# zju3dv/Diffuman4D

Measured on NVIDIA H100. Metric: unet_window_denoise_steps_per_sec, higher is better.
Workload: dtype bf16

## Files before the change

diffuman4d_b200/csrc/common.cuh:

```cuda
#pragma once
#include <cuda.h>
#include <cuda_bf16.h>
#include <cuda_runtime.h>
#include <stdint.h>
#include <string>

namespace d4d {

typedef __nv_bfloat16 bf16;

void set_error(const std::string& msg);
#define D4D_CUDA_OK(expr)                                                                        \
  do {                                                                                           \
    cudaError_t _e = (expr);                                                                     \
    if (_e != cudaSuccess) {                                                                     \
      d4d::set_error(std::string(#expr) + " failed: " + cudaGetErrorString(_e) + " @" + __FILE__ + \
                     ":" + std::to_string(__LINE__));                                            \
      return 2;                                                                                  \
    }                                                                                            \
  } while (0)
#define D4D_REQUIRE(cond, msg)                                                                   \
  do {                                                                                           \
    if (!(cond)) {                                                                               \
      d4d::set_error(std::string("invalid argument: ") + msg + " (" #cond ") @" + __FILE__ + ":" + \
                     std::to_string(__LINE__));                                                  \
      return 1;                                                                                  \
    }                                                                                            \
  } while (0)

int make_tmap_2d(CUtensorMap* out, const void* base, uint64_t rows, uint64_t cols, uint64_t ld,
                 uint32_t box_cols, uint32_t box_rows, int swizzle_bytes);
int make_tmap_nhwc(CUtensorMap* out, const void* base, uint64_t n, uint64_t h, uint64_t w, uint64_t c,
                   uint32_t box_c, uint32_t box_w, uint32_t box_h, uint32_t box_n, int swizzle_bytes, int stride = 1);

#ifdef __CUDACC__
__device__ __forceinline__ uint32_t smem_u32(const void* p) {
  return static_cast<uint32_t>(__cvta_generic_to_shared(p));
}
__device__ __forceinline__ bool elect_one() {
  uint32_t pred = 0;
  asm volatile(
      "{\n\t.reg .b32 rx;\n\t.reg .pred px;\n\t"
      "elect.sync rx|px, 0xffffffff;\n\t"
      "selp.b32 %0, 1, 0, px;\n\t}\n"
      : "=r"(pred));
  return pred != 0;
}

__device__ __forceinline__ void mbar_init(uint64_t* bar, uint32_t count) {
  asm volatile("mbarrier.init.shared::cta.b64 [%0], %1;" ::"r"(smem_u32(bar)), "r"(count) : "memory");
}
__device__ __forceinline__ void fence_mbar_init() {
  asm volatile("fence.mbarrier_init.release.cluster;" ::: "memory");
}
__device__ __forceinline__ void mbar_expect_tx(uint64_t* bar, uint32_t bytes) {
  asm volatile("mbarrier.arrive.expect_tx.shared::cta.b64 _, [%0], %1;" ::"r"(smem_u32(bar)), "r"(bytes)
               : "memory");
}
__device__ __forceinline__ void mbar_arrive(uint64_t* bar) {
  asm volatile("mbarrier.arrive.shared::cta.b64 _, [%0];" ::"r"(smem_u32(bar)) : "memory");
}
__device__ __forceinline__ bool mbar_try_wait(uint64_t* bar, uint32_t parity) {
  uint32_t ok;
  asm volatile(
      "{\n\t.reg .pred p;\n\t"
      "mbarrier.try_wait.parity.shared::cta.b64 p, [%1], %2;\n\t"
      "selp.b32 %0, 1, 0, p;\n\t}\n"
      : "=r"(ok)
      : "r"(smem_u32(bar)), "r"(parity)
      : "memory");
  return ok != 0;
}
#ifndef D4D_SPIN_LIMIT
#define D4D_SPIN_LIMIT (1u << 26)
#endif
__device__ __forceinline__ void mbar_wait(uint64_t* bar, uint32_t parity) {
  uint32_t spins = 0;
  while (!mbar_try_wait(bar, parity)) {
    if (++spins > D4D_SPIN_LIMIT) {
      printf("d4d: mbarrier timeout block=(%d,%d) thread=%d bar=%u parity=%u\n", blockIdx.x, blockIdx.y,
             threadIdx.x, smem_u32(bar), parity);
      __trap();
    }
  }
}

__device__ __forceinline__ void fence_proxy_async_smem() {
  asm volatile("fence.proxy.async.shared::cta;" ::: "memory");
}
__device__ __forceinline__ void named_barrier_sync(int id, int threads) {
  asm volatile("bar.sync %0, %1;" ::"r"(id), "r"(threads) : "memory");
}
__device__ __forceinline__ void st_shared_u32(uint32_t addr, uint32_t v) {
  asm volatile("st.shared.b32 [%0], %1;" ::"r"(addr), "r"(v) : "memory");
}
__device__ __forceinline__ uint32_t ld_shared_u32(uint32_t addr) {
  uint32_t v;
  asm volatile("ld.shared.b32 %0, [%1];" : "=r"(v) : "r"(addr) : "memory");
  return v;
}
__device__ __forceinline__ void pdl_wait() { asm volatile("griddepcontrol.wait;" ::: "memory"); }
__device__ __forceinline__ void pdl_launch_dependents() { asm volatile("griddepcontrol.launch_dependents;" ::: "memory"); }
template <int R> __device__ __forceinline__ void setmaxnreg_dec() { asm volatile("setmaxnreg.dec.sync.aligned.u32 %0;" ::"n"(R)); }
template <int R> __device__ __forceinline__ void setmaxnreg_inc() { asm volatile("setmaxnreg.inc.sync.aligned.u32 %0;" ::"n"(R)); }

__device__ __forceinline__ void tma_prefetch_desc(const CUtensorMap* t) {
  asm volatile("prefetch.tensormap [%0];" ::"l"(reinterpret_cast<uint64_t>(t)) : "memory");
}
__device__ __forceinline__ void tma_load_2d(void* dst, const CUtensorMap* t, uint64_t* bar, int c0, int c1) {
  asm volatile(
      "cp.async.bulk.tensor.2d.shared::cluster.global.tile.mbarrier::complete_tx::bytes [%0], [%1, {%3, %4}], [%2];"
      ::"r"(smem_u32(dst)), "l"(reinterpret_cast<uint64_t>(t)), "r"(smem_u32(bar)), "r"(c0), "r"(c1)
      : "memory");
}
__device__ __forceinline__ void tma_load_4d(void* dst, const CUtensorMap* t, uint64_t* bar, int c0, int c1, int c2,
                                            int c3) {
  asm volatile(
      "cp.async.bulk.tensor.4d.shared::cluster.global.tile.mbarrier::complete_tx::bytes [%0], [%1, {%3, %4, %5, %6}], [%2];"
      ::"r"(smem_u32(dst)), "l"(reinterpret_cast<uint64_t>(t)), "r"(smem_u32(bar)), "r"(c0), "r"(c1), "r"(c2),
      "r"(c3)
      : "memory");
}

__device__ __forceinline__ void tma_store_2d(const CUtensorMap* t, const void* src, int c0, int c1) {
  asm volatile("cp.async.bulk.tensor.2d.global.shared::cta.bulk_group [%0, {%2, %3}], [%1];"
               ::"l"(reinterpret_cast<uint64_t>(t)), "r"(smem_u32(src)), "r"(c0), "r"(c1) : "memory");
}
__device__ __forceinline__ void bulk_commit_group() { asm volatile("cp.async.bulk.commit_group;" ::: "memory"); }
template <int N> __device__ __forceinline__ void bulk_wait_group_read() {
  asm volatile("cp.async.bulk.wait_group.read %0;" ::"n"(N) : "memory");
}
template <int N> __device__ __forceinline__ void bulk_wait_group() {
  asm volatile("cp.async.bulk.wait_group %0;" ::"n"(N) : "memory");
}

__device__ __forceinline__ uint32_t pack_bf16x2(float lo, float hi) {
  __nv_bfloat162 v = __floats2bfloat162_rn(lo, hi);
  return *reinterpret_cast<uint32_t*>(&v);
}
__device__ __forceinline__ float2 unpack_bf16x2(uint32_t u) {
  __nv_bfloat162 v = *reinterpret_cast<__nv_bfloat162*>(&u);
  return __bfloat1622float2(v);
}
__device__ __forceinline__ float silu_f(float x) { return __fdividef(x, 1.0f + __expf(-x)); }
__device__ __forceinline__ float gelu_erf_f(float g) {
  const float u = fabsf(g);
  float q = fmaf(-4.8811754095e-04f, u, 7.1988063864e-03f);
  q = fmaf(q, u, -5.2146803588e-02f);
  q = fmaf(q, u, -4.5959571004e-01f);
  q = fmaf(q, u, -1.1510006189e+00f);
  float e;
  asm("ex2.approx.ftz.f32 %0, %1;" : "=f"(e) : "f"(q * u));
  return fmaf(-0.5f * u, e, fmaxf(g, 0.f));
}
#endif

}
```

diffuman4d_b200/csrc/gemm_wgmma.cu:

```cuda
#include "kernels.h"
#include "wgmma.cuh"

namespace d4d {

namespace {

constexpr int BLOCK_M = 128;
constexpr int BLOCK_K = 64;
constexpr int A_BYTES = BLOCK_M * BLOCK_K * 2;
constexpr int BAR_BYTES = 1024;
constexpr int NUM_THREADS = 384;
constexpr int MAX_SMEM = 227 * 1024;

constexpr int SLAB_COLS = 32;
constexpr int SLAB_BYTES = 64 * SLAB_COLS * 2;

template <int BN, bool kStaged>
struct GemmCfg {
  static constexpr int STAGE_BYTES = A_BYTES + BN * BLOCK_K * 2;
  static constexpr int STAGING_BYTES = kStaged ? 2 * 64 * BN * 2 : 0;
  static constexpr int STAGES_FIT = (MAX_SMEM - 1024 - BAR_BYTES - STAGING_BYTES) / STAGE_BYTES;
  static constexpr int STAGES = STAGES_FIT > 8 ? 8 : STAGES_FIT;
  static constexpr int SMEM = 1024 + BAR_BYTES + STAGES * STAGE_BYTES + STAGING_BYTES;
};

struct TileCoord {
  int m0;
  int n_img0, y0, x0;
  int pa, pb;
};

template <bool kConv>
__device__ __forceinline__ void tile_coords(const GemmKernelArgs& a, int m_tile, TileCoord& t) {
  if (!kConv) {
    t.m0 = m_tile * BLOCK_M;
    t.n_img0 = t.y0 = t.x0 = 0;
    t.pa = t.pb = 0;
  } else {
    const int ph = a.n_phases > 1 ? m_tile / a.tiles_per_phase : 0;
    m_tile -= ph * a.tiles_per_phase;
    t.pa = ph >> 1;
    t.pb = ph & 1;
    int tx = m_tile % a.tiles_x;
    int r = m_tile / a.tiles_x;
    int ty = r % a.tiles_y;
    int tn = r / a.tiles_y;
    t.m0 = 0;
    t.x0 = tx * a.BW;
    t.y0 = ty * a.BH;
    t.n_img0 = tn * a.BN;
  }
}

template <bool kConv>
__device__ __forceinline__ void row_of(const GemmKernelArgs& a, const TileCoord& tc, int rr, long long& row, int& img,
                                       bool& valid) {
  if (!kConv) {
    row = static_cast<long long>(tc.m0) + rr;
    valid = row < a.M;
    img = a.rows_per_image > 0 ? static_cast<int>(row / a.rows_per_image) : 0;
  } else {
    const int bx = rr % a.BW;
    const int r2 = rr / a.BW;
    const int by = r2 % a.BH;
    const int bn = r2 / a.BH;
    const int x = tc.x0 + bx, y = tc.y0 + by, n = tc.n_img0 + bn;
    valid = (x < a.W) && (y < a.H) && (n < a.n_img);
    row = (static_cast<long long>(n) * a.out_H + (y * a.out_sy + a.out_oy + tc.pa)) * a.out_W + (x * a.out_sx + a.out_ox + tc.pb);
    img = n;
  }
}

enum : int { E_BIAS = 1, E_ROWVEC = 2, E_ACT = 4, E_RES = 8, E_STATS = 16, E_KV = 32, E_ALL = 63 };
__host__ __device__ constexpr bool gemm_staged(bool conv, int epi) { return !conv && !(epi & E_KV); }

template <int BN, bool kGeglu, bool kConv, int kEpi>
__global__ void __launch_bounds__(NUM_THREADS, 1)
gemm_wgmma_kernel(const __grid_constant__ CUtensorMap tmap_a, const __grid_constant__ CUtensorMap tmap_a2,
                  const __grid_constant__ CUtensorMap tmap_b, const __grid_constant__ CUtensorMap tmap_c,
                  const __grid_constant__ CUtensorMap tmap_r, const GemmKernelArgs a) {
  constexpr bool kStaged = gemm_staged(kConv, kEpi);
  using Cfg = GemmCfg<BN, kStaged>;
  constexpr int STAGES = Cfg::STAGES;
  extern __shared__ uint8_t smem_raw[];
  uint8_t* smem = reinterpret_cast<uint8_t*>((reinterpret_cast<uintptr_t>(smem_raw) + 1023) & ~uintptr_t(1023));
  uint64_t* full = reinterpret_cast<uint64_t*>(smem);
  uint64_t* empty = full + STAGES;
  uint64_t* res_full = empty + STAGES;
  uint8_t* ring = smem + BAR_BYTES;

  const int warp = __shfl_sync(0xffffffffu, threadIdx.x >> 5, 0);
  const int lane = threadIdx.x & 31;
  const int total_tiles = a.m_tiles * a.n_tiles;

  if (threadIdx.x == 0) {
    tma_prefetch_desc(&tmap_a);
    tma_prefetch_desc(&tmap_b);
    if (a.kb_split < a.k_blocks) tma_prefetch_desc(&tmap_a2);
    for (int i = 0; i < STAGES; ++i) {
      mbar_init(&full[i], 1);
      mbar_init(&empty[i], 2);
    }
    mbar_init(&res_full[0], 1);
    mbar_init(&res_full[1], 1);
    fence_mbar_init();
  }
  __syncthreads();
  pdl_wait();
  pdl_launch_dependents();

  if (warp < 4) {
    setmaxnreg_dec<40>();
    if (threadIdx.x == 0) {
      const uint32_t tx_bytes = A_BYTES + static_cast<uint32_t>(a.block_n) * BLOCK_K * 2;
      int stage = 0;
      uint32_t phase = 0;
      for (int tile = blockIdx.x; tile < total_tiles; tile += gridDim.x) {
        const int m_tile = tile / a.n_tiles;
        const int n_tile = tile % a.n_tiles;
        TileCoord tc;
        tile_coords<kConv>(a, m_tile, tc);
        const int n0 = n_tile * a.block_n;
        for (int kb = 0; kb < a.k_blocks; ++kb) {
          mbar_wait(&empty[stage], phase ^ 1);
          uint8_t* sa = ring + stage * Cfg::STAGE_BYTES;
          uint8_t* sb = sa + A_BYTES;
          mbar_expect_tx(&full[stage], tx_bytes);
          if (!kConv) {
            if (kb < a.kb_split) tma_load_2d(sa, &tmap_a, &full[stage], kb * BLOCK_K, tc.m0);
            else tma_load_2d(sa, &tmap_a2, &full[stage], (kb - a.kb_split) * BLOCK_K, tc.m0);
            tma_load_2d(sb, &tmap_b, &full[stage], kb * BLOCK_K, n0);
          } else {
            const int tap = kb / a.cin_blocks;
            const int cb = kb - tap * a.cin_blocks;
            tma_load_4d(sa, &tmap_a, &full[stage], cb * BLOCK_K, tc.x0 * a.in_stride + a.tap_dx[tap] + tc.pb,
                        tc.y0 * a.in_stride + a.tap_dy[tap] + tc.pa, tc.n_img0);
            tma_load_2d(sb, &tmap_b, &full[stage], tap * a.Cin + cb * BLOCK_K, n0 + (tc.pa * 2 + tc.pb) * a.N);
          }
          if (++stage == STAGES) { stage = 0; phase ^= 1; }
        }
      }
    }
    return;
  }

  setmaxnreg_inc<232>();
  const int wg = (warp >> 2) - 1;
  const int wq = warp & 3;
  const bool wg_leader = (threadIdx.x & 127) == 0;
  const int r_base = wg * 64 + wq * 16 + (lane >> 2);
  const int c_base = 2 * (lane & 3);
  const uint32_t ring_u32 = smem_u32(ring);
  const bool staged = kStaged && a.staged;
  uint8_t* stg = ring + STAGES * Cfg::STAGE_BYTES + wg * 64 * BN * 2;
  const uint32_t stg_u32 = smem_u32(stg) + (r_base - wg * 64) * 64 + c_base * 2;
  const int stg_xor = (lane >> 3) & 3;
  const bool has_res = (kEpi & E_RES) && !kGeglu && a.residual != nullptr;
  const int out_cols = kGeglu ? a.N / 2 : a.N;
  uint32_t res_phase = 0;

  int stage = 0;
  uint32_t phase = 0;
  float acc[BN / 2];
  for (int tile = blockIdx.x; tile < total_tiles; tile += gridDim.x) {
    const int m_tile = tile / a.n_tiles;
    const int n_tile = tile % a.n_tiles;
    TileCoord tc;
    tile_coords<kConv>(a, m_tile, tc);
    const int n0 = n_tile * a.block_n;
    const int ocol0 = kGeglu ? n0 / 2 : n0;
    const int ocols = min(kGeglu ? a.block_n / 2 : a.block_n, out_cols - ocol0);
    const int n_slabs = (ocols + SLAB_COLS - 1) / SLAB_COLS;
    const int orow0 = tc.m0 + wg * 64;
    const bool stg_live = staged && orow0 < a.M;

    int prev_stage = -1;
    for (int kb = 0; kb < a.k_blocks; ++kb) {
      mbar_wait(&full[stage], phase);
      const uint32_t sa = ring_u32 + stage * Cfg::STAGE_BYTES + wg * 64 * 128;
      const uint32_t sb = ring_u32 + stage * Cfg::STAGE_BYTES + A_BYTES;
      const uint64_t adesc = make_wgmma_desc(sa, 16, 1024);
      const uint64_t bdesc = make_wgmma_desc(sb, 16, 1024);
      wgmma_fence();
#pragma unroll
      for (int k = 0; k < BLOCK_K / 16; ++k) {
        const int scale_d = (kb | k) != 0 ? 1 : 0;
        if constexpr (BN == 64) wgmma_ss_n64(acc, adesc + 2 * k, bdesc + 2 * k, scale_d);
        else if constexpr (BN == 128) wgmma_ss_n128(acc, adesc + 2 * k, bdesc + 2 * k, scale_d);
        else if constexpr (BN == 160) wgmma_ss_n160(acc, adesc + 2 * k, bdesc + 2 * k, scale_d);
        else if constexpr (BN == 192) wgmma_ss_n192(acc, adesc + 2 * k, bdesc + 2 * k, scale_d);
        else wgmma_ss_n256(acc, adesc + 2 * k, bdesc + 2 * k, scale_d);
      }
      wgmma_commit();
      if (kb == 0 && staged && wg_leader) {
        bulk_wait_group_read<0>();
        if (has_res && stg_live) {
          mbar_expect_tx(&res_full[wg], n_slabs * SLAB_BYTES);
          for (int s = 0; s < n_slabs; ++s)
            tma_load_2d(stg + s * SLAB_BYTES, &tmap_r, &res_full[wg], ocol0 + s * SLAB_COLS, orow0);
        }
      }
      wgmma_wait<1>();
      if (prev_stage >= 0 && wg_leader) mbar_arrive(&empty[prev_stage]);
      prev_stage = stage;
      if (++stage == STAGES) { stage = 0; phase ^= 1; }
    }
    wgmma_wait<0>();
    wgmma_fence_regs(acc);
    if (wg_leader) mbar_arrive(&empty[prev_stage]);

    long long rows[2];
    int imgs[2];
    bool valid[2];
    row_of<kConv>(a, tc, r_base, rows[0], imgs[0], valid[0]);
    row_of<kConv>(a, tc, r_base + 8, rows[1], imgs[1], valid[1]);
    if (staged) {
      named_barrier_sync(1 + wg, 128);
      if (has_res && stg_live) {
        mbar_wait(&res_full[wg], res_phase);
        res_phase ^= 1;
      }
    }
    auto stg_addr = [&](int j, int h) {
      return stg_u32 + h * 8 * 64 + (j >> 2) * SLAB_BYTES + (((j & 3) ^ stg_xor) << 4);
    };

    if constexpr (kGeglu) {
      const bool has_bias = (kEpi & E_BIAS) && a.bias != nullptr;
#pragma unroll
      for (int p = 0; p < BN / 16; ++p) {
        if (16 * p >= a.block_n || n0 + 16 * p >= a.N) break;
        float2 ba = make_float2(0.f, 0.f), bg = make_float2(0.f, 0.f);
        if (has_bias) {
          ba = __ldg(reinterpret_cast<const float2*>(a.bias + n0 + 16 * p + c_base));
          bg = __ldg(reinterpret_cast<const float2*>(a.bias + n0 + 16 * p + 8 + c_base));
        }
        const int ocol = n0 / 2 + 8 * p + c_base;
#pragma unroll
        for (int h = 0; h < 2; ++h) {
          if (!valid[h]) continue;
          const float a0 = acc[8 * p + 2 * h] + ba.x, a1 = acc[8 * p + 2 * h + 1] + ba.y;
          const float g0 = acc[8 * p + 4 + 2 * h] + bg.x, g1 = acc[8 * p + 4 + 2 * h + 1] + bg.y;
          const uint32_t o = pack_bf16x2(a0 * gelu_erf_f(g0), a1 * gelu_erf_f(g1));
          if (staged) st_shared_u32(stg_addr(p, h), o);
          else *reinterpret_cast<uint32_t*>(a.out + static_cast<size_t>(rows[h]) * a.ldo + ocol) = o;
        }
      }
    } else {
      const bool has_bias = (kEpi & E_BIAS) && a.bias != nullptr, has_rv = (kEpi & E_ROWVEC) && a.rowvec != nullptr;
      const bool has_stats = (kEpi & E_STATS) && a.stats != nullptr;
      const bool has_act = (kEpi & E_ACT) && a.act == 1, has_scale = (kEpi & E_ACT) && a.out_scale != 1.0f;
      const bool has_kv = (kEpi & E_KV) && a.kv_world > 0;
      const long long row0 = __shfl_sync(0xffffffffu, rows[0], 0);
      const bool stats_on = has_stats && __shfl_sync(0xffffffffu, valid[0] ? 1 : 0, 0);
      const int stats_img = !kConv ? static_cast<int>(row0 / a.stats_rows) : __shfl_sync(0xffffffffu, imgs[0], 0);
#pragma unroll
      for (int j = 0; j < BN / 8; ++j) {
        const int cl = 8 * j + c_base;
        const int col = n0 + cl;
        if (8 * j >= a.block_n || n0 + 8 * j >= a.N) break;
        float2 b2 = make_float2(0.f, 0.f);
        if (has_bias) b2 = __ldg(reinterpret_cast<const float2*>(a.bias + col));
        float sv[2][2];
#pragma unroll
        for (int h = 0; h < 2; ++h) {
          sv[h][0] = sv[h][1] = 0.f;
          if (!valid[h]) continue;
          float f0 = acc[4 * j + 2 * h] + b2.x, f1 = acc[4 * j + 2 * h + 1] + b2.y;
          if (has_rv) {
            const float2 v = unpack_bf16x2(*reinterpret_cast<const uint32_t*>(a.rowvec + static_cast<size_t>(imgs[h]) * a.ld_rowvec + col));
            f0 += v.x; f1 += v.y;
          }
          if (has_act) { f0 = silu_f(f0); f1 = silu_f(f1); }
          if (has_scale) { f0 *= a.out_scale; f1 *= a.out_scale; }
          if (has_res) {
            const float2 v = unpack_bf16x2(staged ? ld_shared_u32(stg_addr(j, h))
                                                  : *reinterpret_cast<const uint32_t*>(a.residual + static_cast<size_t>(rows[h]) * a.ld_res + col));
            f0 += v.x; f1 += v.y;
          }
          const uint32_t o = pack_bf16x2(f0, f1);
          if (has_stats) {
            const float2 rv = unpack_bf16x2(o);
            sv[h][0] = rv.x; sv[h][1] = rv.y;
          }
          if (has_kv && col >= a.kv_col0) {
            const long long half = rows[h] / a.kv_rows_local;
            const long long grow = half * a.kv_rows_global + a.kv_row_offset + (rows[h] - half * a.kv_rows_local);
            const size_t off = static_cast<size_t>(grow) * a.kv_ld + (col - a.kv_col0);
#pragma unroll 1
            for (int rk = 0; rk < a.kv_world; ++rk) *reinterpret_cast<uint32_t*>(a.kv_dst[rk] + off) = o;
          } else if (staged) {
            st_shared_u32(stg_addr(j, h), o);
          } else {
            *reinterpret_cast<uint32_t*>(a.out + static_cast<size_t>(rows[h]) * a.ldo + col) = o;
          }
        }
        if (has_stats) {
          float s0 = sv[0][0] + sv[1][0], s1 = sv[0][1] + sv[1][1];
          float q0 = sv[0][0] * sv[0][0] + sv[1][0] * sv[1][0], q1 = sv[0][1] * sv[0][1] + sv[1][1] * sv[1][1];
#pragma unroll
          for (int m = 4; m < 32; m <<= 1) {
            s0 += __shfl_xor_sync(0xffffffffu, s0, m);
            s1 += __shfl_xor_sync(0xffffffffu, s1, m);
            q0 += __shfl_xor_sync(0xffffffffu, q0, m);
            q1 += __shfl_xor_sync(0xffffffffu, q1, m);
          }
          if (stats_on && lane < 4) {
            unsigned long long* st = reinterpret_cast<unsigned long long*>(a.stats) + (static_cast<size_t>(stats_img) * a.N + col) * 2;
            atomicAdd(st + 0, static_cast<unsigned long long>(__float2ll_rn(s0 * kGnSumScale)));
            atomicAdd(st + 1, static_cast<unsigned long long>(__float2ll_rn(q0 * kGnSqScale)));
            atomicAdd(st + 2, static_cast<unsigned long long>(__float2ll_rn(s1 * kGnSumScale)));
            atomicAdd(st + 3, static_cast<unsigned long long>(__float2ll_rn(q1 * kGnSqScale)));
          }
        }
      }
    }
    if (staged) {
      fence_proxy_async_smem();
      named_barrier_sync(1 + wg, 128);
      if (wg_leader && stg_live) {
        for (int s = 0; s < n_slabs; ++s) tma_store_2d(&tmap_c, stg + s * SLAB_BYTES, ocol0 + s * SLAB_COLS, orow0);
        bulk_commit_group();
      }
    }
  }
  if (staged && wg_leader) bulk_wait_group<0>();
}

}

int gemm_prepare(const GemmDesc& d, GemmLaunch* L) {
  D4D_REQUIRE(d.N % 16 == 0, "GEMM N must be a multiple of 16");
  D4D_REQUIRE(d.out != nullptr && d.A != nullptr && d.Wt != nullptr, "null operand");
  D4D_REQUIRE(d.kv_world >= 0 && d.kv_world <= 8, "K/V scatter: world must be in [1, 8]");
  if (d.kv_world > 0) {
    D4D_REQUIRE(!d.conv && !d.geglu && d.kv_col0 >= 0 && d.kv_col0 < d.N && d.kv_col0 % 16 == 0 && d.kv_ld % 8 == 0 &&
                d.kv_ld >= d.N - d.kv_col0, "K/V scatter arguments");
    for (int r = 0; r < d.kv_world; ++r) D4D_REQUIRE(d.kv_dst[r] != nullptr, "K/V scatter: null destination buffer");
    D4D_REQUIRE(d.kv_rows_local > 0 && d.M % d.kv_rows_local == 0, "K/V scatter: M must be a multiple of rows_local");
    D4D_REQUIRE(d.kv_row_offset >= 0 && d.kv_row_offset + d.kv_rows_local <= d.kv_rows_global,
                "K/V scatter: row_offset + rows_local exceeds rows_global");
  }
  GemmKernelArgs& a = L->args;
  memset(&a, 0, sizeof(a));
  int dev = 0, sms = 0;
  D4D_CUDA_OK(cudaGetDevice(&dev));
  D4D_CUDA_OK(cudaDeviceGetAttribute(&sms, cudaDevAttrMultiProcessorCount, dev));
  int bn = d.block_n;
  if (bn <= 0) {
    const long long rows = d.conv ? static_cast<long long>(d.n_img) * d.H * d.W : d.M;
    const long long m_tiles_est = (rows + BLOCK_M - 1) / BLOCK_M;
    long long best_cost = -1;
    for (int c : {64, 128, 160, 192, 256}) {
      if (d.geglu && c % 64 != 0) continue;
      const long long tiles = m_tiles_est * ((d.N + c - 1) / c);
      const long long waves = (tiles + sms - 1) / sms;
      const long long cost = waves * (c + 64) + (static_cast<long long>((d.N + c - 1) / c) * c - d.N) / 4;
      if (best_cost < 0 || cost <= best_cost) { best_cost = cost; bn = c; }
    }
  }
  D4D_REQUIRE(bn >= 16 && bn <= 256 && bn % 16 == 0 && (d.block_n <= 0 || d.N % bn == 0), "no valid block_n");
  a.block_n = bn;
  a.n_tiles = (d.N + bn - 1) / bn;
  a.N = d.N;
  a.bias = d.bias;
  a.rowvec = d.rowvec;
  a.ld_rowvec = d.ld_rowvec;
  a.rows_per_image = d.rows_per_image;
  a.residual = d.residual;
  a.ld_res = d.ld_res;
  a.out = d.out;
  a.ldo = d.ldo;
  a.geglu = d.geglu;
  a.act = d.act;
  a.out_scale = d.out_scale;
  a.stats = d.stats;
  a.stats_rows = d.stats_rows > 0 ? d.stats_rows : 1;
  D4D_REQUIRE(d.stats == nullptr || (!d.geglu && d.kv_world == 0), "GroupNorm statistics: plain / conv epilogue only");
  D4D_REQUIRE(d.stats == nullptr || d.conv || (d.stats_rows > 0 && d.stats_rows % 32 == 0), "statistics need rows-per-image % 32 == 0");
  D4D_REQUIRE(d.stats == nullptr || d.conv || d.M % d.stats_rows == 0, "statistics need M % rows-per-image == 0");
  a.kv_world = d.kv_world;
  a.kv_col0 = d.kv_col0;
  a.kv_ld = d.kv_ld;
  a.kv_rows_local = d.kv_rows_local > 0 ? d.kv_rows_local : 1;
  a.kv_rows_global = d.kv_rows_global;
  a.kv_row_offset = d.kv_row_offset;
  for (int i = 0; i < 8; ++i) a.kv_dst[i] = d.kv_dst[i];
  D4D_REQUIRE(d.ldo % 8 == 0 && (d.residual == nullptr || d.ld_res % 8 == 0) &&
              (d.rowvec == nullptr || d.ld_rowvec % 8 == 0), "leading dimensions must be multiples of 8");

  if (!d.conv) {
    D4D_REQUIRE(d.K1 > 0 && d.K1 % 8 == 0 && d.K2 % 8 == 0, "K must be a multiple of 8");
    D4D_REQUIRE(d.A2 == nullptr || d.K1 % BLOCK_K == 0, "two-source GEMM needs K1 % 64 == 0");
    a.mode = 0;
    a.M = d.M;
    a.m_tiles = (d.M + BLOCK_M - 1) / BLOCK_M;
    a.kb_split = (d.K1 + BLOCK_K - 1) / BLOCK_K;
    const int kb2 = d.A2 ? (d.K2 + BLOCK_K - 1) / BLOCK_K : 0;
    a.k_blocks = a.kb_split + kb2;
    const int K = d.K1 + (d.A2 ? d.K2 : 0);
    if (int rc = make_tmap_2d(&L->tmap_a, d.A, d.M, d.K1, d.lda, BLOCK_K, BLOCK_M, 128)) return rc;
    if (d.A2) {
      if (int rc = make_tmap_2d(&L->tmap_a2, d.A2, d.M, d.K2, d.lda2, BLOCK_K, BLOCK_M, 128)) return rc;
    } else {
      L->tmap_a2 = L->tmap_a;
    }
    if (int rc = make_tmap_2d(&L->tmap_b, d.Wt, d.N, K, K, BLOCK_K, bn, 128)) return rc;
    const auto aligned16 = [](const void* p) { return (reinterpret_cast<uintptr_t>(p) & 15) == 0; };
    a.staged = d.kv_world == 0 && (d.geglu ? bn % (2 * SLAB_COLS) : bn % SLAB_COLS) == 0 && aligned16(d.out) &&
               (d.residual == nullptr || aligned16(d.residual));
    L->tmap_c = L->tmap_r = L->tmap_a;
    if (a.staged) {
      if (int rc = make_tmap_2d(&L->tmap_c, d.out, d.M, d.geglu ? d.N / 2 : d.N, d.ldo, SLAB_COLS, 64, 64)) return rc;
      if (d.residual && !d.geglu)
        if (int rc = make_tmap_2d(&L->tmap_r, d.residual, d.M, d.N, d.ld_res, SLAB_COLS, 64, 64)) return rc;
    }
  } else {
    D4D_REQUIRE(d.Cin % 8 == 0, "conv Cin must be a multiple of 8");
    D4D_REQUIRE(d.conv_kind >= 0 && d.conv_kind <= 3, "conv_kind");
    D4D_REQUIRE(d.conv_kind != 1 || (d.H % 2 == 0 && d.W % 2 == 0), "stride-2 conv needs even H, W");
    a.mode = 1;
    a.n_img = d.n_img; a.Cin = d.Cin;
    a.in_stride = 1; a.out_sy = a.out_sx = 1; a.out_oy = a.out_ox = 0;
    a.n_phases = 1;
    if (d.conv_kind >= 2) {
      const int pa = d.conv_kind == 3 ? 0 : d.up_a, pb = d.conv_kind == 3 ? 0 : d.up_b;
      a.n_taps = 4;
      for (int t = 0; t < 4; ++t) {
        a.tap_dy[t] = static_cast<signed char>((t >> 1) + pa - 1);
        a.tap_dx[t] = static_cast<signed char>((t & 1) + pb - 1);
      }
      a.H = d.H; a.W = d.W; a.out_H = 2 * d.H; a.out_W = 2 * d.W;
      a.out_sy = a.out_sx = 2; a.out_oy = pa; a.out_ox = pb;
      if (d.conv_kind == 3) a.n_phases = 4;
    } else {
      a.n_taps = 9;
      for (int t = 0; t < 9; ++t) {
        a.tap_dy[t] = static_cast<signed char>(t / 3 - 1);
        a.tap_dx[t] = static_cast<signed char>(t % 3 - 1);
      }
      if (d.conv_kind == 1) { a.in_stride = 2; a.H = d.H / 2; a.W = d.W / 2; }
      else { a.H = d.H; a.W = d.W; }
      a.out_H = a.H; a.out_W = a.W;
    }
    a.M = d.n_img * a.H * a.W;
    a.cin_blocks = (d.Cin + BLOCK_K - 1) / BLOCK_K;
    a.k_blocks = a.n_taps * a.cin_blocks;
    a.kb_split = a.k_blocks;
    int bw = 16; while (bw > a.W) bw >>= 1;
    int bh = 128 / bw; while (bh > a.H && bh > 1) bh >>= 1;
    int bnimg = 128 / (bw * bh);
    D4D_REQUIRE(bw * bh * bnimg == 128 && bnimg <= 256, "conv tile shape");
    D4D_REQUIRE(d.stats == nullptr || (bw * bh) % 32 == 0, "statistics need 32-row warps inside one image");
    a.BW = bw; a.BH = bh; a.BN = bnimg;
    a.tiles_x = (a.W + bw - 1) / bw;
    a.tiles_y = (a.H + bh - 1) / bh;
    const int tiles_n = (d.n_img + bnimg - 1) / bnimg;
    a.tiles_per_phase = a.tiles_x * a.tiles_y * tiles_n;
    a.m_tiles = a.tiles_per_phase * a.n_phases;
    a.M *= a.n_phases;
    if (int rc = make_tmap_nhwc(&L->tmap_a, d.A, d.n_img, d.H, d.W, d.Cin, BLOCK_K, bw, bh, bnimg, 128, a.in_stride)) return rc;
    L->tmap_a2 = L->tmap_c = L->tmap_r = L->tmap_a;
    const uint64_t kw = static_cast<uint64_t>(a.n_taps) * d.Cin;
    if (int rc = make_tmap_2d(&L->tmap_b, d.Wt, static_cast<uint64_t>(d.N) * a.n_phases, kw, kw, BLOCK_K, bn, 128)) return rc;
  }
  const int total = a.m_tiles * a.n_tiles;
  L->grid = total < sms ? total : sms;
  return 0;
}

namespace {

using GemmKernelFn = void (*)(const CUtensorMap, const CUtensorMap, const CUtensorMap, const CUtensorMap,
                              const CUtensorMap, const GemmKernelArgs);
struct GemmVariant {
  int bn;
  bool geglu, conv;
  int epi;
  GemmKernelFn fn;
  int smem;
};
#define D4D_GV(BN, G, C, E) {BN, G, C, E, gemm_wgmma_kernel<BN, G, C, E>, GemmCfg<BN, gemm_staged(C, E)>::SMEM}
#define D4D_GV_PLAIN(BN)                                                                                              \
                                         \
  D4D_GV(BN, false, false, 0), D4D_GV(BN, false, false, E_BIAS), D4D_GV(BN, false, false, E_BIAS | E_RES),           \
  D4D_GV(BN, false, false, E_BIAS | E_RES | E_STATS), D4D_GV(BN, false, false, E_ALL)
#define D4D_GV_CONV(BN)                                                                                               \
                                                            \
  D4D_GV(BN, false, true, E_BIAS | E_ROWVEC | E_STATS), D4D_GV(BN, false, true, E_BIAS | E_RES | E_STATS),           \
  D4D_GV(BN, false, true, E_BIAS | E_STATS), D4D_GV(BN, false, true, E_ALL)
const GemmVariant kGemmVariants[] = {
    D4D_GV_PLAIN(128), D4D_GV_CONV(128), D4D_GV(128, true, false, E_BIAS),
    D4D_GV_PLAIN(160), D4D_GV_CONV(160),
    D4D_GV_PLAIN(192),
    D4D_GV_PLAIN(256), D4D_GV_CONV(256), D4D_GV(256, true, false, E_BIAS),
    D4D_GV(64, false, false, E_ALL), D4D_GV(64, false, true, E_ALL), D4D_GV(64, true, false, E_BIAS),
};
#undef D4D_GV_CONV
#undef D4D_GV_PLAIN
#undef D4D_GV
constexpr int kNumGemmVariants = sizeof(kGemmVariants) / sizeof(kGemmVariants[0]);

int gemm_variant_at(const GemmKernelArgs& a, int bn) {
  const bool conv = a.mode != 0, geglu = a.geglu != 0;
  int need = 0;
  if (a.bias) need |= E_BIAS;
  if (!geglu) {
    if (a.rowvec) need |= E_ROWVEC;
    if (a.act == 1 || a.out_scale != 1.0f) need |= E_ACT;
    if (a.residual) need |= E_RES;
    if (a.stats) need |= E_STATS;
    if (a.kv_world > 0) need |= E_KV;
  }
  int generic = -1;
  for (int i = 0; i < kNumGemmVariants; ++i) {
    const GemmVariant& v = kGemmVariants[i];
    if (v.bn != bn || v.geglu != geglu || v.conv != conv) continue;
    if (v.epi == need) return i;
    if ((v.epi & need) == need && (generic < 0 || v.epi == E_ALL)) generic = i;
  }
  return generic;
}

int gemm_variant_of(const GemmKernelArgs& a) {
  for (int bn : {64, 128, 160, 192, 256}) {
    if (bn < a.block_n) continue;
    const int vi = gemm_variant_at(a, bn);
    if (vi >= 0) return vi;
  }
  return -1;
}

}

int gemm_run(const GemmLaunch& L, cudaStream_t stream) {
  static PerDeviceOnce attr_once[kNumGemmVariants];
  const int vi = gemm_variant_of(L.args);
  D4D_REQUIRE(vi >= 0, "no GEMM kernel instantiation covers this launch");
  const GemmVariant& v = kGemmVariants[vi];
  if (int rc = ensure_dyn_smem(v.fn, v.smem, attr_once[vi])) return rc;
  D4D_CUDA_OK(launch_pdl(v.fn, dim3(L.grid), dim3(NUM_THREADS), v.smem, stream, L.tmap_a, L.tmap_a2, L.tmap_b, L.tmap_c, L.tmap_r,
                         L.args));
  D4D_CUDA_OK(cudaGetLastError());
  return 0;
}

double gemm_flops(const GemmLaunch& L) {
  return 2.0 * static_cast<double>(L.args.M) * L.args.N * (static_cast<double>(L.args.k_blocks) * BLOCK_K);
}

}
```

diffuman4d_b200/csrc/kernels.h:

```cpp
#pragma once
#include <cstdlib>
#include <mutex>
#include <utility>
#include <string.h>

#include "common.cuh"

namespace d4d {

constexpr float kGnSumScale = 268435456.f;
constexpr float kGnSqScale = 16777216.f;

struct GemmKernelArgs {
  int M, N, k_blocks, block_n, n_tiles, m_tiles;
  int mode;
  int kb_split;
  int H, W, n_img, Cin, cin_blocks, BW, BH, BN, tiles_x, tiles_y;
  int n_taps, in_stride, out_sy, out_sx, out_oy, out_ox, out_H, out_W;
  int n_phases, tiles_per_phase;
  signed char tap_dy[9], tap_dx[9];
  const float* bias;
  const bf16* rowvec;
  int ld_rowvec, rows_per_image;
  const bf16* residual;
  int ld_res;
  bf16* out;
  int ldo;
  int staged;
  int geglu;
  int act;
  float out_scale;
  long long* stats;
  int stats_rows;
  int kv_world, kv_col0, kv_ld;
  long long kv_rows_local, kv_rows_global, kv_row_offset;
  bf16* kv_dst[8];
};

struct GemmDesc {
  const bf16* A = nullptr;
  int lda = 0, K1 = 0;
  const bf16* A2 = nullptr;
  int lda2 = 0, K2 = 0;
  const bf16* Wt = nullptr;
  int M = 0, N = 0;
  const float* bias = nullptr;
  const bf16* rowvec = nullptr;
  int ld_rowvec = 0, rows_per_image = 0;
  const bf16* residual = nullptr;
  int ld_res = 0;
  bf16* out = nullptr;
  int ldo = 0;
  int geglu = 0;
  int act = 0;
  float out_scale = 1.0f;
  int block_n = 0;
  long long* stats = nullptr;
  int stats_rows = 0;
  int kv_world = 0, kv_col0 = 0, kv_ld = 0;
  long long kv_rows_local = 0, kv_rows_global = 0, kv_row_offset = 0;
  bf16* kv_dst[8] = {nullptr, nullptr, nullptr, nullptr, nullptr, nullptr, nullptr, nullptr};
  int conv = 0, n_img = 0, H = 0, W = 0, Cin = 0;
  int conv_kind = 0, up_a = 0, up_b = 0;
};

struct GemmLaunch {
  CUtensorMap tmap_a, tmap_a2, tmap_b, tmap_c, tmap_r;
  GemmKernelArgs args;
  int grid;
};

int gemm_prepare(const GemmDesc& d, GemmLaunch* L);
int gemm_run(const GemmLaunch& L, cudaStream_t stream);
double gemm_flops(const GemmLaunch& L);

struct AttnDesc {
  const bf16* q = nullptr;
  const bf16* k = nullptr;
  const bf16* v = nullptr;
  int ld_qkv = 0;
  bf16* out = nullptr;
  int ld_out = 0;
  int batch = 0, seq = 0, heads = 0, head_dim = 0;
  int seq_kv = 0;
  int ld_kv = 0;
  float scale = 0.f;
};
struct AttnLaunch {
  CUtensorMap tmap_q, tmap_k, tmap_v;
  AttnDesc d;
  int grid_x, grid_y;
  int variant;
};
int attn_prepare(const AttnDesc& d, AttnLaunch* L);
int attn_run(const AttnLaunch& L, cudaStream_t stream);
double attn_flops(const AttnDesc& d);

int groupnorm_stats_run(const bf16* x, int C, int n_img, int hw, long long* stats, cudaStream_t stream);
int groupnorm_apply_run(const bf16* x1, int C1, const long long* stats1, const bf16* x2, int C2, const long long* stats2, int n_img,
                        int hw, int groups, float eps, const float* gamma, const float* beta, int silu, bf16* out,
                        cudaStream_t stream);
int layernorm_run(const bf16* x, int rows, int C, float eps, const float* gamma, const float* beta, bf16* out,
                  cudaStream_t stream);

int sinusoid_run(const float* pos, int n, int dim, int flip, float freq_shift, bf16* out, cudaStream_t stream);
int sinusoid_i64_run(const long long* pos, int n, int dim, int flip, float freq_shift, bf16* out, cudaStream_t stream);
int silu_run(const bf16* x, long long n, bf16* out, cudaStream_t stream);
int im2col_nchw_run(const bf16* x, int n, int Cin, int H, int W, int cin_pad, int KP, bf16* out, cudaStream_t stream);
int nhwc_to_nchw_run(const bf16* x, int ld, int n, int C, int hw, bf16* out, cudaStream_t stream);
int pose_conv0_run(const bf16* x_nchw, int n, int H, int W, const bf16* w, const float* bias, bf16* out_nhwc4,
                   cudaStream_t stream);
int pose_conv_run(const bf16* x, int n, int Cin, int H, int W, const bf16* w, const float* bias, int Cout, int ksize,
                  int stride, bf16* out_nhwc, cudaStream_t stream);
int im2col_nhwc_run(const bf16* x, int n, int H, int W, int C, int ksize, int stride, bf16* out, cudaStream_t stream);

struct AssembleArgs {
  bf16* latents;
  const bf16* pixel;
  const bf16* plucker;
  const bf16* skel_latents;
  const bf16* mask;
  const long long* timestep_indices;
  const long long* timesteps_table;
  int n_steps;
  int F, h, w, cfg;
  bf16* sample;
  long long* timestep_out;
};
int assemble_input_run(const AssembleArgs& a, cudaStream_t stream);

struct DdimArgs {
  const bf16* noise;
  const bf16* latents;
  const bf16* mask;
  const long long* timestep_indices;
  const long long* timesteps_table;
  const float* alphas_cumprod;
  int n_steps, T;
  float final_alpha_cumprod;
  int F, chw, hw, cfg;
  float guidance;
  int prediction_type;
  int clip_sample;
  float clip_range;
  int emulate_bf16;
  bf16* out;
};
int cfg_ddim_step_run(const DdimArgs& a, long long* ts_out, cudaStream_t stream);

constexpr int kDpmCoefs = 6;
struct DpmArgs {
  const bf16* noise;
  const bf16* latents;
  const bf16* mask;
  const long long* timestep_indices;
  const float* coefs;
  int n_steps;
  int F, chw, hw, cfg;
  float guidance;
  int prediction_type;
  int solver_order;
  int final_first_order;
  int emulate_bf16;
  bf16* x0_prev;
  const int* lower_order_nums;
  int* lower_order_nums_out;
  bf16* out;
};
int cfg_dpm_step_run(const DpmArgs& a, long long* ts_out, cudaStream_t stream);

constexpr int kUniPCCoefs = 14;
struct UniPCArgs {
  const bf16* noise;
  const bf16* latents;
  const bf16* mask;
  const long long* timestep_indices;
  const float* coefs;
  int n_steps;
  int F, chw, hw, cfg;
  float guidance;
  int prediction_type;
  int solver_order;
  int emulate_bf16;
  bf16* x0_prev;
  bf16* x0_prev2;
  bf16* last_sample;
  const int* lower_order_nums;
  int* lower_order_nums_out;
  bf16* out;
};
int cfg_unipc_step_run(const UniPCArgs& a, long long* ts_out, cudaStream_t stream);

struct KvFlagArgs {
  unsigned int* flags[8];
  int rank, world;
  unsigned int epoch;
  int slot;
};
int kv_signal_run(const KvFlagArgs& a, cudaStream_t stream);
int kv_wait_run(const KvFlagArgs& a, cudaStream_t stream);

struct WindowResultLayout {
  size_t x0, ts, lon, bytes;
};
inline WindowResultLayout window_result_layout(long long F_total, long long chw, bool dpm) {
  WindowResultLayout L;
  const size_t rows = static_cast<size_t>(F_total) * static_cast<size_t>(chw) * 2;
  L.x0 = rows;
  L.ts = dpm ? 2 * rows : rows;
  L.lon = L.ts + static_cast<size_t>(F_total) * 8;
  L.bytes = L.lon + (dpm ? static_cast<size_t>(F_total) * 4 : 0);
  return L;
}
struct WindowScatterArgs {
  void* dst[8];
  int world, rank, F_local, F_total;
  long long chw;
  const bf16* latents;
  const long long* ts;
  const bf16* x0_prev;
  const int* lower_order_nums;
};
int window_scatter_run(const WindowScatterArgs& a, size_t dst_bytes, cudaStream_t stream);

struct PerDeviceOnce {
  std::once_flag flag[64];
};
template <typename F>
inline int ensure_dyn_smem(F func, int bytes, PerDeviceOnce& once) {
  int dev = 0;
  D4D_CUDA_OK(cudaGetDevice(&dev));
  if (dev < 0 || dev >= 64) return 0;
  cudaError_t err = cudaSuccess;
  std::call_once(once.flag[dev], [&] { err = cudaFuncSetAttribute(func, cudaFuncAttributeMaxDynamicSharedMemorySize, bytes); });
  D4D_CUDA_OK(err);
  return 0;
}

inline bool pdl_enabled() { return false; }
template <typename... KArgs, typename... Args>
inline cudaError_t launch_pdl(void (*kernel)(KArgs...), dim3 grid, dim3 block, size_t smem, cudaStream_t stream, Args&&... args) {
  cudaLaunchConfig_t cfg = {};
  cfg.gridDim = grid;
  cfg.blockDim = block;
  cfg.dynamicSmemBytes = smem;
  cfg.stream = stream;
  cudaLaunchAttribute attr[1];
  attr[0].id = cudaLaunchAttributeProgrammaticStreamSerialization;
  attr[0].val.programmaticStreamSerializationAllowed = pdl_enabled() ? 1 : 0;
  cfg.attrs = attr;
  cfg.numAttrs = 1;
  return cudaLaunchKernelEx(&cfg, kernel, std::forward<Args>(args)...);
}

}
```

Baseline: 13.23.

## Pair conv GEMM CTAs in 2-CTA clusters and multicast the weight tile

Conv GEMMs now launch as 2-CTA clusters. The two CTAs take adjacent M tiles with the same N tile, and each loads half of the shared B (weight) tile with TMA multicast into both CTAs' shared memory. Empty barriers count arrivals from both CTAs through remote mbarrier arrives, and the producer drains the remaining stages before exit. Grid sizing and block_n selection now use the occupancy API's max active clusters instead of the SM count. The aim is to halve global/L2 weight traffic, at the cost of cross-CTA coupling, cluster scheduling limits, and padding tiles_per_phase for the 4-phase case.

Measured after the change: 13.32 (median of 6 runs). About the same (+0.7%).

```diff
diff --git a/diffuman4d_b200/csrc/common.cuh b/diffuman4d_b200/csrc/common.cuh
--- a/diffuman4d_b200/csrc/common.cuh
+++ b/diffuman4d_b200/csrc/common.cuh
@@ -60,6 +60,14 @@
 __device__ __forceinline__ void mbar_arrive(uint64_t* bar) {
   asm volatile("mbarrier.arrive.shared::cta.b64 _, [%0];" ::"r"(smem_u32(bar)) : "memory");
 }
+__device__ __forceinline__ void mbar_arrive_cluster(uint64_t* bar, uint32_t rank) {
+  asm volatile(
+      "{\n\t.reg .b32 ra;\n\t"
+      "mapa.shared::cluster.u32 ra, %0, %1;\n\t"
+      "mbarrier.arrive.shared::cluster.b64 _, [ra];\n\t}\n"
+      ::"r"(smem_u32(bar)), "r"(rank)
+      : "memory");
+}
 __device__ __forceinline__ bool mbar_try_wait(uint64_t* bar, uint32_t parity) {
   uint32_t ok;
   asm volatile(
@@ -101,6 +109,29 @@
 }
 __device__ __forceinline__ void pdl_wait() { asm volatile("griddepcontrol.wait;" ::: "memory"); }
 __device__ __forceinline__ void pdl_launch_dependents() { asm volatile("griddepcontrol.launch_dependents;" ::: "memory"); }
+__device__ __forceinline__ uint32_t cluster_ctarank() {
+  uint32_t r;
+  asm volatile("mov.u32 %0, %%cluster_ctarank;" : "=r"(r));
+  return r;
+}
+__device__ __forceinline__ uint32_t cluster_nctarank() {
+  uint32_t r;
+  asm volatile("mov.u32 %0, %%cluster_nctarank;" : "=r"(r));
+  return r;
+}
+__device__ __forceinline__ uint32_t cluster_id_x() {
+  uint32_t r;
+  asm volatile("mov.u32 %0, %%clusterid.x;" : "=r"(r));
+  return r;
+}
+__device__ __forceinline__ uint32_t cluster_count_x() {
+  uint32_t r;
+  asm volatile("mov.u32 %0, %%nclusterid.x;" : "=r"(r));
+  return r;
+}
+__device__ __forceinline__ void cluster_sync() {
+  asm volatile("barrier.cluster.arrive.release;\n\tbarrier.cluster.wait.acquire;" ::: "memory");
+}
 template <int R> __device__ __forceinline__ void setmaxnreg_dec() { asm volatile("setmaxnreg.dec.sync.aligned.u32 %0;" ::"n"(R)); }
 template <int R> __device__ __forceinline__ void setmaxnreg_inc() { asm volatile("setmaxnreg.inc.sync.aligned.u32 %0;" ::"n"(R)); }
 
@@ -119,6 +150,13 @@
       "cp.async.bulk.tensor.4d.shared::cluster.global.tile.mbarrier::complete_tx::bytes [%0], [%1, {%3, %4, %5, %6}], [%2];"
       ::"r"(smem_u32(dst)), "l"(reinterpret_cast<uint64_t>(t)), "r"(smem_u32(bar)), "r"(c0), "r"(c1), "r"(c2),
       "r"(c3)
+      : "memory");
+}
+__device__ __forceinline__ void tma_load_2d_multicast(void* dst, const CUtensorMap* t, uint64_t* bar, int c0, int c1,
+                                                      uint16_t cta_mask) {
+  asm volatile(
+      "cp.async.bulk.tensor.2d.shared::cluster.global.tile.mbarrier::complete_tx::bytes.multicast::cluster [%0], [%1, {%3, %4}], [%2], %5;"
+      ::"r"(smem_u32(dst)), "l"(reinterpret_cast<uint64_t>(t)), "r"(smem_u32(bar)), "r"(c0), "r"(c1), "h"(cta_mask)
       : "memory");
 }
 
diff --git a/diffuman4d_b200/csrc/gemm_wgmma.cu b/diffuman4d_b200/csrc/gemm_wgmma.cu
--- a/diffuman4d_b200/csrc/gemm_wgmma.cu
+++ b/diffuman4d_b200/csrc/gemm_wgmma.cu
@@ -91,7 +91,8 @@
 
   const int warp = __shfl_sync(0xffffffffu, threadIdx.x >> 5, 0);
   const int lane = threadIdx.x & 31;
-  const int total_tiles = a.m_tiles * a.n_tiles;
+  const int cs = static_cast<int>(cluster_nctarank());
+  const int pair_tiles = (a.m_tiles + cs - 1) / cs * a.n_tiles;
 
   if (threadIdx.x == 0) {
     tma_prefetch_desc(&tmap_a);
@@ -99,13 +100,13 @@
     if (a.kb_split < a.k_blocks) tma_prefetch_desc(&tmap_a2);
     for (int i = 0; i < STAGES; ++i) {
       mbar_init(&full[i], 1);
-      mbar_init(&empty[i], 2);
+      mbar_init(&empty[i], 2 * cs);
     }
     mbar_init(&res_full[0], 1);
     mbar_init(&res_full[1], 1);
     fence_mbar_init();
   }
-  __syncthreads();
+  cluster_sync();
   pdl_wait();
   pdl_launch_dependents();
 
@@ -113,30 +114,41 @@
     setmaxnreg_dec<40>();
     if (threadIdx.x == 0) {
       const uint32_t tx_bytes = A_BYTES + static_cast<uint32_t>(a.block_n) * BLOCK_K * 2;
+      const int rank = static_cast<int>(cluster_ctarank());
+      const int b_rows = a.block_n / cs;
       int stage = 0;
       uint32_t phase = 0;
-      for (int tile = blockIdx.x; tile < total_tiles; tile += gridDim.x) {
-        const int m_tile = tile / a.n_tiles;
-        const int n_tile = tile % a.n_tiles;
+      for (int pt = cluster_id_x(); pt < pair_tiles; pt += cluster_count_x()) {
+        const int m_tile = pt / a.n_tiles * cs + rank;
+        const int n_tile = pt % a.n_tiles;
         TileCoord tc;
         tile_coords<kConv>(a, m_tile, tc);
-        const int n0 = n_tile * a.block_n;
+        const int b_row0 = n_tile * a.block_n + rank * b_rows + (tc.pa * 2 + tc.pb) * a.N;
         for (int kb = 0; kb < a.k_blocks; ++kb) {
           mbar_wait(&empty[stage], phase ^ 1);
           uint8_t* sa = ring + stage * Cfg::STAGE_BYTES;
-          uint8_t* sb = sa + A_BYTES;
+          uint8_t* sb = sa + A_BYTES + rank * b_rows * BLOCK_K * 2;
           mbar_expect_tx(&full[stage], tx_bytes);
+          int kw;
           if (!kConv) {
             if (kb < a.kb_split) tma_load_2d(sa, &tmap_a, &full[stage], kb * BLOCK_K, tc.m0);
             else tma_load_2d(sa, &tmap_a2, &full[stage], (kb - a.kb_split) * BLOCK_K, tc.m0);
-            tma_load_2d(sb, &tmap_b, &full[stage], kb * BLOCK_K, n0);
+            kw = kb * BLOCK_K;
           } else {
             const int tap = kb / a.cin_blocks;
             const int cb = kb - tap * a.cin_blocks;
             tma_load_4d(sa, &tmap_a, &full[stage], cb * BLOCK_K, tc.x0 * a.in_stride + a.tap_dx[tap] + tc.pb,
                         tc.y0 * a.in_stride + a.tap_dy[tap] + tc.pa, tc.n_img0);
-            tma_load_2d(sb, &tmap_b, &full[stage], tap * a.Cin + cb * BLOCK_K, n0 + (tc.pa * 2 + tc.pb) * a.N);
+            kw = tap * a.Cin + cb * BLOCK_K;
           }
+          if (cs == 1) tma_load_2d(sb, &tmap_b, &full[stage], kw, b_row0);
+          else tma_load_2d_multicast(sb, &tmap_b, &full[stage], kw, b_row0, static_cast<uint16_t>((1u << cs) - 1));
+          if (++stage == STAGES) { stage = 0; phase ^= 1; }
+        }
+      }
+      if (cs > 1) {
+        for (int i = 0; i < STAGES; ++i) {
+          mbar_wait(&empty[stage], phase ^ 1);
           if (++stage == STAGES) { stage = 0; phase ^= 1; }
         }
       }
@@ -162,9 +174,13 @@
   int stage = 0;
   uint32_t phase = 0;
   float acc[BN / 2];
-  for (int tile = blockIdx.x; tile < total_tiles; tile += gridDim.x) {
-    const int m_tile = tile / a.n_tiles;
-    const int n_tile = tile % a.n_tiles;
+  auto release = [&](int s) {
+    mbar_arrive_cluster(&empty[s], 0);
+    if (cluster_nctarank() > 1) mbar_arrive_cluster(&empty[s], 1);
+  };
+  for (int pt = cluster_id_x(); pt < pair_tiles; pt += cluster_count_x()) {
+    const int m_tile = pt / a.n_tiles * static_cast<int>(cluster_nctarank()) + static_cast<int>(cluster_ctarank());
+    const int n_tile = pt % a.n_tiles;
     TileCoord tc;
     tile_coords<kConv>(a, m_tile, tc);
     const int n0 = n_tile * a.block_n;
@@ -201,13 +217,13 @@
         }
       }
       wgmma_wait<1>();
-      if (prev_stage >= 0 && wg_leader) mbar_arrive(&empty[prev_stage]);
+      if (prev_stage >= 0 && wg_leader) release(prev_stage);
       prev_stage = stage;
       if (++stage == STAGES) { stage = 0; phase ^= 1; }
     }
     wgmma_wait<0>();
     wgmma_fence_regs(acc);
-    if (wg_leader) mbar_arrive(&empty[prev_stage]);
+    if (wg_leader) release(prev_stage);
 
     long long rows[2];
     int imgs[2];
@@ -327,6 +343,8 @@
   if (staged && wg_leader) bulk_wait_group<0>();
 }
 
+int gemm_max_clusters(int cs, int* clusters);
+
 }
 
 int gemm_prepare(const GemmDesc& d, GemmLaunch* L) {
@@ -343,18 +361,18 @@
   }
   GemmKernelArgs& a = L->args;
   memset(&a, 0, sizeof(a));
-  int dev = 0, sms = 0;
-  D4D_CUDA_OK(cudaGetDevice(&dev));
-  D4D_CUDA_OK(cudaDeviceGetAttribute(&sms, cudaDevAttrMultiProcessorCount, dev));
   int bn = d.block_n;
   if (bn <= 0) {
-    const long long rows = d.conv ? static_cast<long long>(d.n_img) * d.H * d.W : d.M;
+    const long long rows = d.conv ? static_cast<long long>(d.n_img) * d.H * d.W * (d.conv_kind == 3 ? 4 : 1) : d.M;
     const long long m_tiles_est = (rows + BLOCK_M - 1) / BLOCK_M;
+    const int cs = d.conv && m_tiles_est >= 2 ? 2 : 1;
+    int clusters = 0;
+    if (int rc = gemm_max_clusters(cs, &clusters)) return rc;
     long long best_cost = -1;
     for (int c : {64, 128, 160, 192, 256}) {
       if (d.geglu && c % 64 != 0) continue;
-      const long long tiles = m_tiles_est * ((d.N + c - 1) / c);
-      const long long waves = (tiles + sms - 1) / sms;
+      const long long tiles = (m_tiles_est + cs - 1) / cs * ((d.N + c - 1) / c);
+      const long long waves = (tiles + clusters - 1) / clusters;
       const long long cost = waves * (c + 64) + (static_cast<long long>((d.N + c - 1) / c) * c - d.N) / 4;
       if (best_cost < 0 || cost <= best_cost) { best_cost = cost; bn = c; }
     }
@@ -389,6 +407,7 @@
   D4D_REQUIRE(d.ldo % 8 == 0 && (d.residual == nullptr || d.ld_res % 8 == 0) &&
               (d.rowvec == nullptr || d.ld_rowvec % 8 == 0), "leading dimensions must be multiples of 8");
 
+  uint64_t b_rows = 0, b_cols = 0;
   if (!d.conv) {
     D4D_REQUIRE(d.K1 > 0 && d.K1 % 8 == 0 && d.K2 % 8 == 0, "K must be a multiple of 8");
     D4D_REQUIRE(d.A2 == nullptr || d.K1 % BLOCK_K == 0, "two-source GEMM needs K1 % 64 == 0");
@@ -405,7 +424,8 @@
     } else {
       L->tmap_a2 = L->tmap_a;
     }
-    if (int rc = make_tmap_2d(&L->tmap_b, d.Wt, d.N, K, K, BLOCK_K, bn, 128)) return rc;
+    b_rows = d.N;
+    b_cols = K;
     const auto aligned16 = [](const void* p) { return (reinterpret_cast<uintptr_t>(p) & 15) == 0; };
     a.staged = d.kv_world == 0 && (d.geglu ? bn % (2 * SLAB_COLS) : bn % SLAB_COLS) == 0 && aligned16(d.out) &&
                (d.residual == nullptr || aligned16(d.residual));
@@ -457,15 +477,20 @@
     a.tiles_y = (a.H + bh - 1) / bh;
     const int tiles_n = (d.n_img + bnimg - 1) / bnimg;
     a.tiles_per_phase = a.tiles_x * a.tiles_y * tiles_n;
+    if (a.n_phases == 4) a.tiles_per_phase += a.tiles_per_phase & 1;
     a.m_tiles = a.tiles_per_phase * a.n_phases;
     a.M *= a.n_phases;
     if (int rc = make_tmap_nhwc(&L->tmap_a, d.A, d.n_img, d.H, d.W, d.Cin, BLOCK_K, bw, bh, bnimg, 128, a.in_stride)) return rc;
     L->tmap_a2 = L->tmap_c = L->tmap_r = L->tmap_a;
-    const uint64_t kw = static_cast<uint64_t>(a.n_taps) * d.Cin;
-    if (int rc = make_tmap_2d(&L->tmap_b, d.Wt, static_cast<uint64_t>(d.N) * a.n_phases, kw, kw, BLOCK_K, bn, 128)) return rc;
-  }
-  const int total = a.m_tiles * a.n_tiles;
-  L->grid = total < sms ? total : sms;
+    b_rows = static_cast<uint64_t>(d.N) * a.n_phases;
+    b_cols = static_cast<uint64_t>(a.n_taps) * d.Cin;
+  }
+  L->cs = d.conv && a.m_tiles >= 2 ? 2 : 1;
+  if (int rc = make_tmap_2d(&L->tmap_b, d.Wt, b_rows, b_cols, b_cols, BLOCK_K, bn / L->cs, 128)) return rc;
+  int clusters = 0;
+  if (int rc = gemm_max_clusters(L->cs, &clusters)) return rc;
+  const int pair_tiles = (a.m_tiles + L->cs - 1) / L->cs * a.n_tiles;
+  L->grid = L->cs * (pair_tiles < clusters ? pair_tiles : clusters);
   return 0;
 }
 
@@ -531,16 +556,45 @@
   return -1;
 }
 
+PerDeviceOnce attr_once[kNumGemmVariants];
+
+int gemm_max_clusters(int cs, int* clusters) {
+  static PerDeviceOnce once[2];
+  static int count[2][64];
+  int dev = 0;
+  D4D_CUDA_OK(cudaGetDevice(&dev));
+  D4D_REQUIRE(cs >= 1 && cs <= 2 && dev >= 0 && dev < 64, "cluster size / device ordinal");
+  const GemmVariant& v = kGemmVariants[0];
+  if (int rc = ensure_dyn_smem(v.fn, v.smem, attr_once[0])) return rc;
+  cudaError_t err = cudaSuccess;
+  std::call_once(once[cs - 1].flag[dev], [&] {
+    cudaLaunchConfig_t cfg = {};
+    cfg.gridDim = dim3(cs);
+    cfg.blockDim = dim3(NUM_THREADS);
+    cfg.dynamicSmemBytes = v.smem;
+    cudaLaunchAttribute attr;
+    attr.id = cudaLaunchAttributeClusterDimension;
+    attr.val.clusterDim.x = cs;
+    attr.val.clusterDim.y = attr.val.clusterDim.z = 1;
+    cfg.attrs = &attr;
+    cfg.numAttrs = 1;
+    err = cudaOccupancyMaxActiveClusters(&count[cs - 1][dev], reinterpret_cast<const void*>(v.fn), &cfg);
+  });
+  D4D_CUDA_OK(err);
+  *clusters = count[cs - 1][dev];
+  D4D_REQUIRE(*clusters > 0, "the device holds no cluster of the GEMM kernel");
+  return 0;
+}
+
 }
 
 int gemm_run(const GemmLaunch& L, cudaStream_t stream) {
-  static PerDeviceOnce attr_once[kNumGemmVariants];
   const int vi = gemm_variant_of(L.args);
   D4D_REQUIRE(vi >= 0, "no GEMM kernel instantiation covers this launch");
   const GemmVariant& v = kGemmVariants[vi];
   if (int rc = ensure_dyn_smem(v.fn, v.smem, attr_once[vi])) return rc;
-  D4D_CUDA_OK(launch_pdl(v.fn, dim3(L.grid), dim3(NUM_THREADS), v.smem, stream, L.tmap_a, L.tmap_a2, L.tmap_b, L.tmap_c, L.tmap_r,
-                         L.args));
+  D4D_CUDA_OK(launch_pdl(v.fn, LaunchGrid(dim3(L.grid), L.cs), dim3(NUM_THREADS), v.smem, stream, L.tmap_a, L.tmap_a2, L.tmap_b,
+                         L.tmap_c, L.tmap_r, L.args));
   D4D_CUDA_OK(cudaGetLastError());
   return 0;
 }
diff --git a/diffuman4d_b200/csrc/kernels.h b/diffuman4d_b200/csrc/kernels.h
--- a/diffuman4d_b200/csrc/kernels.h
+++ b/diffuman4d_b200/csrc/kernels.h
@@ -68,6 +68,7 @@
   CUtensorMap tmap_a, tmap_a2, tmap_b, tmap_c, tmap_r;
   GemmKernelArgs args;
   int grid;
+  int cs;
 };
 
 int gemm_prepare(const GemmDesc& d, GemmLaunch* L);
@@ -238,18 +239,27 @@
 }
 
 inline bool pdl_enabled() { return false; }
+struct LaunchGrid {
+  dim3 grid;
+  unsigned cluster;
+  LaunchGrid(dim3 g, unsigned c = 1) : grid(g), cluster(c) {}
+};
 template <typename... KArgs, typename... Args>
-inline cudaError_t launch_pdl(void (*kernel)(KArgs...), dim3 grid, dim3 block, size_t smem, cudaStream_t stream, Args&&... args) {
+inline cudaError_t launch_pdl(void (*kernel)(KArgs...), LaunchGrid grid, dim3 block, size_t smem, cudaStream_t stream, Args&&... args) {
   cudaLaunchConfig_t cfg = {};
-  cfg.gridDim = grid;
+  cfg.gridDim = grid.grid;
   cfg.blockDim = block;
   cfg.dynamicSmemBytes = smem;
   cfg.stream = stream;
-  cudaLaunchAttribute attr[1];
+  cudaLaunchAttribute attr[2];
   attr[0].id = cudaLaunchAttributeProgrammaticStreamSerialization;
   attr[0].val.programmaticStreamSerializationAllowed = pdl_enabled() ? 1 : 0;
+  attr[1].id = cudaLaunchAttributeClusterDimension;
+  attr[1].val.clusterDim.x = grid.cluster;
+  attr[1].val.clusterDim.y = 1;
+  attr[1].val.clusterDim.z = 1;
   cfg.attrs = attr;
-  cfg.numAttrs = 1;
+  cfg.numAttrs = grid.cluster > 1 ? 2 : 1;
   return cudaLaunchKernelEx(&cfg, kernel, std::forward<Args>(args)...);
 }
 
```
